# rainerzufalldererste/simd_dct

Hardware: AMD Instinct MI355X
Metric: Mpixels/s 8x8 fwd+inv int16 DCT, 8192x8192 plane (higher is better)
Workload: dtype f32

## Files before the change

simd_dct_amd/csrc/huffman_rows.h:

```cpp
#pragma once
#include <hip/hip_runtime.h>
#include "wg_sync.h"
#include <stdint.h>

namespace mdct
{

struct HuffArgs
{
  const int16_t *levels;
  const uint8_t *runs, *counts;
  uint8_t *out;
  uint32_t *seg_bytes;
  size_t seg_stride;
  uint32_t bpr, by0;
  uint32_t dc[12];
  uint32_t ac[256];
};

constexpr uint32_t kHuffRing = 2048;

__device__ __forceinline__ uint32_t ff_bytes(uint32_t w)
{
  const uint32_t t = ~w;
  return ~(((t & 0x7F7F7F7Fu) + 0x7F7F7F7Fu) | t | 0x7F7F7F7Fu);
}

struct HuffTok
{
  uint32_t bits, len;
};

__device__ __forceinline__ HuffTok huff_dc_token(int diff, const uint32_t *dc)
{
  diff = diff > 2047 ? 2047 : (diff < -2047 ? -2047 : diff);
  const int s = diff ? 32 - __builtin_clz((uint32_t)(diff < 0 ? -diff : diff)) : 0;
  const uint32_t e = dc[s];
  return {((e & 0xFFFFu) << s) | ((uint32_t)(diff < 0 ? diff - 1 : diff) & ((1u << s) - 1u)), (e >> 16) + (uint32_t)s};
}

__device__ __forceinline__ HuffTok huff_ac_token(int r, int l, const uint32_t *ac)
{
  l = l > 1023 ? 1023 : (l < -1023 ? -1023 : l);
  const int amp = l + (l >> 31);
  int lead;
  asm("v_ffbh_i32 %0, %1" : "=v"(lead) : "v"(amp));
  const int s = 32 - lead;
  const uint32_t e = ac[(r << 4) | s];
  return {((e & 0xFFFFu) << s) | ((uint32_t)amp & ((1u << s) - 1u)), (e >> 16) + (uint32_t)s};
}

template <int WAVES, int STAGE, bool TAIL, bool LATE_DC>
struct HuffRowCoder
{
  const uint32_t *ac, *dc;
  uint32_t *ring;
  uint32_t (*tot)[WAVES];
  int (*dcx)[2][WAVES];
  uint32_t *out_w;
  uint32_t zrl, eob;
  uint32_t bpr;
  uint32_t base_bits = 0;
  uint32_t par = 0;
  int carry_dc = 0;

  __device__ __forceinline__ void chunk(uint32_t c0, uint32_t *rec, int n, bool live, int prev_dc, const int16_t *lv_g, const uint8_t *rn_g)
  {
    constexpr uint32_t kChunk = 64 * WAVES;
    const uint32_t tid = threadIdx.x, lane = tid & 63, wave = tid >> 6;
    const int nl = n < STAGE ? n : STAGE;
    const uint32_t e0 = rec[0];
// ... 144 lines not shown
          put(eob & 0xFFFFu, eob >> 16);
        if (nacc && widx - win < kHuffRing)
          atomicOr(&ring[widx & (kHuffRing - 1)], acc << (32 - nacc));
      }
      wg_sync();
      const uint32_t stop = min(w_end, win + kHuffRing);
      for (uint32_t w = win + tid; w < stop; w += kChunk)
      {
        out_w[w] = __builtin_bswap32(ring[w & (kHuffRing - 1)]);
        ring[w & (kHuffRing - 1)] = 0;
      }
    }
    base_bits = end_bits;
    par ^= 1;
  }

  __device__ __forceinline__ uint32_t finish()
  {
    const uint32_t rem = base_bits & 31;
    if (rem)
    {
      const uint32_t pad = (8 - (rem & 7)) & 7;
      uint32_t w = ring[(base_bits >> 5) & (kHuffRing - 1)];
      if (pad)
        w |= ((1u << pad) - 1u) << (32 - rem - pad);
      out_w[base_bits >> 5] = __builtin_bswap32(w);
    }
    return (base_bits + 7) / 8;
  }
};

constexpr int kRec16Row = 66;

__device__ __forceinline__ HuffTok huff_ac_token12(uint32_t e, const uint32_t *ac)
{
  int l;
  asm("v_bfe_i32 %0, %1, 0, 12" : "=v"(l) : "v"(e));
  const int amp = l + (l >> 31);
  int lead;
  asm("v_ffbh_i32 %0, %1" : "=v"(lead) : "v"(amp));
  const int s = l ? 32 - lead : 0;
  const uint32_t c = ac[((e >> 12) << 4) | (uint32_t)s];
  return {((c & 0xFFFFu) << s) | ((uint32_t)amp & ((1u << s) - 1u)), (c >> 16) + (uint32_t)s};
}

template <int WAVES, uint32_t RING>
struct HuffRowCoder16
{
  const uint32_t *ac, *dc;
  uint32_t *ring;
  uint32_t (*tot)[WAVES];
  int (*dcx)[2][WAVES];
  uint32_t *out_w;
  uint32_t eob;
  uint32_t bpr;
  uint32_t base_bits = 0;
  uint32_t par = 0;
  int carry_dc = 0;
  uint32_t ff = 0;

  __device__ __forceinline__ void chunk(uint32_t c0, const uint16_t *rec, int n, bool live, int my_dc, bool need_eob)
  {
    constexpr uint32_t kChunk = 64 * WAVES;
    const uint32_t tid = threadIdx.x, lane = tid & 63, wave = tid >> 6;
    const uint32_t *rec2 = reinterpret_cast<const uint32_t *>(rec);
    if (!live)
    {
      my_dc = 0;
      n = 0;
    }
    const int up = __shfl_up(my_dc, 1, 64);
    HuffTok dct = huff_dc_token(my_dc - up, dc);
    if (lane == 0)
      dcx[par][0][wave] = my_dc;
    if (lane == 63)
      dcx[par][1][wave] = my_dc;
    uint32_t bits = 0;
    if (live)
    {
      bits = lane ? dct.len : 0u;
      for (int i = 0; i < n; i += 2)
      {
        const uint32_t w = rec2[i >> 1];
        bits += huff_ac_token12(w & 0xFFFFu, ac).len;
        if (i + 1 < n)
          bits += huff_ac_token12(w >> 16, ac).len;
      }
      if (need_eob)
        bits += eob >> 16;
    }
    uint32_t incl = bits;
#pragma unroll
    for (int d = 1; d < 64; d <<= 1)
    {
      const uint32_t v = __shfl_up(incl, d, 64);
      if (lane >= (uint32_t)d)
        incl += v;
    }
    if (lane == 63)
      tot[par][wave] = incl;
    wg_sync();
    uint32_t wave_start = 0, chunk_bits = 0, lane0_len = 0;
#pragma unroll
    for (uint32_t w = 0; w < (uint32_t)WAVES; w++)
    {
      const int pred = w == 0 ? (c0 == 0 ? 0 : carry_dc) : dcx[par][1][w - 1];
      const HuffTok t0 = huff_dc_token(dcx[par][0][w] - pred, dc);
      const uint32_t l0 = c0 + 64 * w < bpr ? t0.len : 0u;
      const uint32_t t = tot[par][w] + l0;
      if (w == wave)
      {
        lane0_len = l0;
        if (lane == 0)
          dct = t0;
      }
      wave_start += w < wave ? t : 0;
      chunk_bits += t;
    }
    carry_dc = dcx[par][1][WAVES - 1];
    const uint32_t end_bits = base_bits + chunk_bits;
    const uint32_t w_first = base_bits >> 5, w_end = end_bits >> 5;
    for (uint32_t win = w_first; win <= w_end; win += RING)
    {
      if (win != w_first)
      {
        wg_sync();
      }
      if (live)
      {
        const uint32_t cur = base_bits + wave_start + (incl - bits) + (lane ? lane0_len : 0u);
        uint32_t widx = cur >> 5;
        uint32_t acc = 0;
        uint32_t nacc = cur & 31;
        auto put = [&](uint32_t tok, uint32_t len) {
          const uint32_t total = nacc + len;
          if (total < 32)
          {
            acc = (acc << len) | tok;
            nacc = total;
          }
          else
          {
            const uint32_t over = total - 32;
            if (widx - win < RING)
              atomicOr(&ring[widx & (RING - 1)], (acc << ((32 - nacc) & 31)) | (tok >> over));
            widx++;
            acc = tok & ((1u << over) - 1u);
            nacc = over;
          }
        };
        put(dct.bits, dct.len);
        for (int i = 0; i < n; i += 2)
        {
          const uint32_t w = rec2[i >> 1];
          const HuffTok ta = huff_ac_token12(w & 0xFFFFu, ac);
          put(ta.bits, ta.len);
          if (i + 1 < n)
          {
            const HuffTok tb = huff_ac_token12(w >> 16, ac);
            put(tb.bits, tb.len);
          }
        }
        if (need_eob)
          put(eob & 0xFFFFu, eob >> 16);
        if (nacc && widx - win < RING)
          atomicOr(&ring[widx & (RING - 1)], acc << (32 - nacc));
      }
      wg_sync();
      const uint32_t stop = min(w_end, win + RING);
      for (uint32_t w = win + tid; w < stop; w += kChunk)
      {
        const uint32_t v = ring[w & (RING - 1)];
        ff += (uint32_t)__builtin_popcount(ff_bytes(v));
        out_w[w] = __builtin_bswap32(v);
        ring[w & (RING - 1)] = 0;
      }
    }
    base_bits = end_bits;
    par ^= 1;
  }

  __device__ __forceinline__ uint32_t finish(uint32_t *ff_last)
  {
    const uint32_t rem = base_bits & 31;
    *ff_last = 0;
    if (rem)
    {
      const uint32_t pad = (8 - (rem & 7)) & 7;
      uint32_t w = ring[(base_bits >> 5) & (RING - 1)];
      if (pad)
        w |= ((1u << pad) - 1u) << (32 - rem - pad);
      out_w[base_bits >> 5] = __builtin_bswap32(w);
      const uint32_t nbytes = (rem + 7) / 8;
      *ff_last = (uint32_t)__builtin_popcount(ff_bytes(w) & (0xFFFFFFFFu << (8 * (4 - nbytes))));
    }
    return (base_bits + 7) / 8;
  }
};

template <int WAVES, uint32_t RING>
struct HuffSeqCoder16
{
  uint32_t *ring;
  uint32_t (*tot)[WAVES];
  uint32_t *out_w;
  uint32_t base_bits = 0;
  uint32_t par = 0;
  uint32_t ff = 0;

  __device__ __forceinline__ void chunk(const uint16_t *rec, int n, bool live, int my_dc, int pred_dc, bool need_eob, const uint32_t *ac, const uint32_t *dc)
  {
    constexpr uint32_t kChunk = 64 * WAVES;
    const uint32_t tid = threadIdx.x, lane = tid & 63, wave = tid >> 6;
    const uint32_t *rec2 = reinterpret_cast<const uint32_t *>(rec);
    if (!live)
    {
      my_dc = pred_dc = 0;
      n = 0;
    }
    const HuffTok dct = huff_dc_token(my_dc - pred_dc, dc);
    const uint32_t eob = ac[0x00];
    uint32_t bits = 0;
    if (live)
    {
      bits = dct.len;
      for (int i = 0; i < n; i += 2)
      {
        const uint32_t w = rec2[i >> 1];
        bits += huff_ac_token12(w & 0xFFFFu, ac).len;
        if (i + 1 < n)
          bits += huff_ac_token12(w >> 16, ac).len;
      }
      if (need_eob)
        bits += eob >> 16;
    }
    uint32_t incl = bits;
#pragma unroll
    for (int d = 1; d < 64; d <<= 1)
    {
      const uint32_t v = __shfl_up(incl, d, 64);
      if (lane >= (uint32_t)d)
        incl += v;
    }
    if (lane == 63)
      tot[par][wave] = incl;
    wg_sync();
    uint32_t wave_start = 0, chunk_bits = 0;
#pragma unroll
    for (uint32_t w = 0; w < (uint32_t)WAVES; w++)
    {
      const uint32_t t = tot[par][w];
      wave_start += w < wave ? t : 0;
      chunk_bits += t;
    }
    const uint32_t end_bits = base_bits + chunk_bits;
    const uint32_t w_first = base_bits >> 5, w_end = end_bits >> 5;
    for (uint32_t win = w_first; win <= w_end; win += RING)
    {
      if (win != w_first)
        wg_sync();
      if (live)
      {
        const uint32_t cur = base_bits + wave_start + (incl - bits);
        uint32_t widx = cur >> 5;
        uint32_t acc = 0;
        uint32_t nacc = cur & 31;
        auto put = [&](uint32_t tok, uint32_t len) {
          const uint32_t total = nacc + len;
          if (total < 32)
          {
            acc = (acc << len) | tok;
            nacc = total;
          }
          else
          {
            const uint32_t over = total - 32;
            if (widx - win < RING)
              atomicOr(&ring[widx & (RING - 1)], (acc << ((32 - nacc) & 31)) | (tok >> over));
            widx++;
            acc = tok & ((1u << over) - 1u);
            nacc = over;
          }
        };
        put(dct.bits, dct.len);
        for (int i = 0; i < n; i += 2)
        {
          const uint32_t w = rec2[i >> 1];
          const HuffTok ta = huff_ac_token12(w & 0xFFFFu, ac);
          put(ta.bits, ta.len);
          if (i + 1 < n)
          {
            const HuffTok tb = huff_ac_token12(w >> 16, ac);
            put(tb.bits, tb.len);
          }
        }
        if (need_eob)
          put(eob & 0xFFFFu, eob >> 16);
        if (nacc && widx - win < RING)
          atomicOr(&ring[widx & (RING - 1)], acc << (32 - nacc));
      }
      wg_sync();
      const uint32_t stop = min(w_end, win + RING);
      for (uint32_t w = win + tid; w < stop; w += kChunk)
      {
        const uint32_t v = ring[w & (RING - 1)];
        ff += (uint32_t)__builtin_popcount(ff_bytes(v));
        out_w[w] = __builtin_bswap32(v);
        ring[w & (RING - 1)] = 0;
      }
    }
    base_bits = end_bits;
    par ^= 1;
  }

  __device__ __forceinline__ uint32_t finish(uint32_t *ff_last)
  {
    const uint32_t rem = base_bits & 31;
    *ff_last = 0;
    if (rem)
    {
      const uint32_t pad = (8 - (rem & 7)) & 7;
      uint32_t w = ring[(base_bits >> 5) & (RING - 1)];
      if (pad)
        w |= ((1u << pad) - 1u) << (32 - rem - pad);
      out_w[base_bits >> 5] = __builtin_bswap32(w);
      const uint32_t nbytes = (rem + 7) / 8;
      *ff_last = (uint32_t)__builtin_popcount(ff_bytes(w) & (0xFFFFFFFFu << (8 * (4 - nbytes))));
    }
    return (base_bits + 7) / 8;
  }
};

// ... 2 lines not shown
```

simd_dct_amd/csrc/mdct_kernels.hip:

```cpp
#include <hip/hip_runtime.h>
#include <stddef.h>
#include <stdint.h>
#include <stdlib.h>

#include <type_traits>

#include "wg_sync.h"
#include "huffman_rows.h"
#include "pack_rows.h"
#include "mdct_kernels.h"
#include "scan_records.h"
#include "aan_passes.h"

#pragma clang fp contract(off)

namespace mdct
{


enum { K_AVX = 0, K_SSE = 1, K_TRUE = 2 };

__device__ __forceinline__ void aan_fwd8(const DctConsts &C, float &p0, float &p1, float &p2, float &p3, float &p4, float &p5, float &p6, float &p7)
{
  const float t0 = p0 + p7, t7 = p0 - p7, t1 = p1 + p6, t6 = p1 - p6;
// ... 809 lines not shown
__device__ __forceinline__ void quant_dequant8(const AanPk &K, f32x2 (&p)[8], const f32x2 (&qf)[8], const f32x2 (&dq)[8])
{
#define MDCT_Q8(OP, A, B, MOD) OP " %0, %0, " A "0" B MOD OP " %1, %1, " A "1" B MOD OP " %2, %2, " A "2" B MOD OP " %3, %3, " A "3" B MOD OP " %4, %4, " A "4" B MOD OP " %5, %5, " A "5" B MOD OP " %6, %6, " A "6" B MOD OP " %7, %7, " A "7" B MOD
  asm("v_pk_fma_f32 %0, %0, %8, %24 op_sel:[0,0,0] op_sel_hi:[1,1,0]\n\t"
      "v_pk_fma_f32 %1, %1, %9, %24 op_sel:[0,0,0] op_sel_hi:[1,1,0]\n\t"
      "v_pk_fma_f32 %2, %2, %10, %24 op_sel:[0,0,0] op_sel_hi:[1,1,0]\n\t"
      "v_pk_fma_f32 %3, %3, %11, %24 op_sel:[0,0,0] op_sel_hi:[1,1,0]\n\t"
      "v_pk_fma_f32 %4, %4, %12, %24 op_sel:[0,0,0] op_sel_hi:[1,1,0]\n\t"
      "v_pk_fma_f32 %5, %5, %13, %24 op_sel:[0,0,0] op_sel_hi:[1,1,0]\n\t"
      "v_pk_fma_f32 %6, %6, %14, %24 op_sel:[0,0,0] op_sel_hi:[1,1,0]\n\t"
      "v_pk_fma_f32 %7, %7, %15, %24 op_sel:[0,0,0] op_sel_hi:[1,1,0]\n\t"
      "v_pk_add_f32 %0, %0, %24 op_sel:[0,0] op_sel_hi:[1,0] neg_lo:[0,1] neg_hi:[0,1]\n\t"
      "v_pk_add_f32 %1, %1, %24 op_sel:[0,0] op_sel_hi:[1,0] neg_lo:[0,1] neg_hi:[0,1]\n\t"
      "v_pk_add_f32 %2, %2, %24 op_sel:[0,0] op_sel_hi:[1,0] neg_lo:[0,1] neg_hi:[0,1]\n\t"
      "v_pk_add_f32 %3, %3, %24 op_sel:[0,0] op_sel_hi:[1,0] neg_lo:[0,1] neg_hi:[0,1]\n\t"
      "v_pk_add_f32 %4, %4, %24 op_sel:[0,0] op_sel_hi:[1,0] neg_lo:[0,1] neg_hi:[0,1]\n\t"
      "v_pk_add_f32 %5, %5, %24 op_sel:[0,0] op_sel_hi:[1,0] neg_lo:[0,1] neg_hi:[0,1]\n\t"
      "v_pk_add_f32 %6, %6, %24 op_sel:[0,0] op_sel_hi:[1,0] neg_lo:[0,1] neg_hi:[0,1]\n\t"
      "v_pk_add_f32 %7, %7, %24 op_sel:[0,0] op_sel_hi:[1,0] neg_lo:[0,1] neg_hi:[0,1]\n\t"
      "v_pk_mul_f32 %0, %0, %16 op_sel:[0,0] op_sel_hi:[1,1]\n\t"
      "v_pk_mul_f32 %1, %1, %17 op_sel:[0,0] op_sel_hi:[1,1]\n\t"
      "v_pk_mul_f32 %2, %2, %18 op_sel:[0,0] op_sel_hi:[1,1]\n\t"
      "v_pk_mul_f32 %3, %3, %19 op_sel:[0,0] op_sel_hi:[1,1]\n\t"
      "v_pk_mul_f32 %4, %4, %20 op_sel:[0,0] op_sel_hi:[1,1]\n\t"
      "v_pk_mul_f32 %5, %5, %21 op_sel:[0,0] op_sel_hi:[1,1]\n\t"
      "v_pk_mul_f32 %6, %6, %22 op_sel:[0,0] op_sel_hi:[1,1]\n\t"
      "v_pk_mul_f32 %7, %7, %23 op_sel:[0,0] op_sel_hi:[1,1]"
      : "+v"(p[0]), "+v"(p[1]), "+v"(p[2]), "+v"(p[3]), "+v"(p[4]), "+v"(p[5]), "+v"(p[6]), "+v"(p[7])
      : "s"(qf[0]), "s"(qf[1]), "s"(qf[2]), "s"(qf[3]), "s"(qf[4]), "s"(qf[5]), "s"(qf[6]), "s"(qf[7]), "s"(dq[0]), "s"(dq[1]), "s"(dq[2]), "s"(dq[3]), "s"(dq[4]), "s"(dq[5]),
        "s"(dq[6]), "s"(dq[7]), "v"(K.magic));
#undef MDCT_Q8
}

template <bool HAS_LUT, class Rows, bool PRIO = false, bool SAT = true>
__device__ __forceinline__ void i16_roundtrip_rows(const DctConsts &C, const Rows rows, kbytes_t tbp);

__device__ __forceinline__ kbytes_t const_bytes(const void *p)
{
  const uint64_t v = (uint64_t)p;
  const uint32_t lo = __builtin_amdgcn_readfirstlane((uint32_t)v), hi = __builtin_amdgcn_readfirstlane((uint32_t)(v >> 32));
  return (kbytes_t)(((uint64_t)hi << 32) | lo);
}

template <bool SAT>
__device__ __forceinline__ void quant_dequant_pairs(const AanPk &K, f32x2 (&p)[8], karg_pairs_t tq, karg_pairs_t td)
{
  if constexpr (!SAT)
  {
    const f32x2 qf[8] = {tq[0], tq[1], tq[2], tq[3], tq[4], tq[5], tq[6], tq[7]}, dq[8] = {td[0], td[1], td[2], td[3], td[4], td[5], td[6], td[7]};
    quant_dequant8(K, p, qf, dq);
  }
  else
  {
    const f32x2 magic_v = K.magic;
#pragma unroll
    for (int v = 0; v < 8; v++)
    {
      const f32x2 qf = tq[v], dq = td[v];
      f32x2 m;
      MDCT_PKF(m, p[v], qf, magic_v, "op_sel:[0,0,0] op_sel_hi:[1,1,0]");
      if constexpr (SAT)
      {
        m.x = __builtin_amdgcn_fmed3f(m.x, kQLo, kQHi);
        m.y = __builtin_amdgcn_fmed3f(m.y, kQLo, kQHi);
      }
      MDCT_PKA(m, m, K.magic, MDCT_K_LL " " MDCT_NEG_B);
      MDCT_PKM(p[v], m, dq, MDCT_K_LH);
    }
  }
}

template <bool HAS_LUT, class Rows, bool PRIO, bool SAT>
__device__ __forceinline__ void i16_roundtrip_rows(const DctConsts &C, const Rows rows, kbytes_t tbp)
{
  const AanPk &K = reinterpret_cast<const AanPk &>(C);
  uint4 in[8];
#pragma unroll
  for (int r = 0; r < 8; r++)
    in[r] = rows.ld(r);
  MDCT_PHASE_PRIO(1);
  f32x2 P[4][8];
#pragma unroll
  for (int r = 0; r < 8; r++)
  {
    const f32x2 a01 = {(float)(int16_t)(in[r].x & 0xFFFF), (float)(int16_t)(in[r].x >> 16)};
    const f32x2 a23 = {(float)(int16_t)(in[r].y & 0xFFFF), (float)(int16_t)(in[r].y >> 16)};
    const f32x2 a45 = {(float)(int16_t)(in[r].z & 0xFFFF), (float)(int16_t)(in[r].z >> 16)};
    const f32x2 a67 = {(float)(int16_t)(in[r].w & 0xFFFF), (float)(int16_t)(in[r].w >> 16)};
    aan_fwd_h(K, a01, a23, a45, a67, P[0][r], P[1][r], P[2][r], P[3][r]);
  }
  MDCT_PHASE_PRIO(2);
#pragma unroll
  for (int j = 0; j < 4; j++)
  {
    aan_fwd_v(K, P[j]);
    if constexpr (HAS_LUT)
    {
      karg_pairs_t tq = (karg_pairs_t)(tbp + offsetof(OwnTables, qf)) + j * 8, td = (karg_pairs_t)(tbp + offsetof(OwnTables, dq)) + j * 8;
      asm volatile("" : "+s"(tq), "+s"(td));
      quant_dequant_pairs<SAT>(K, P[j], tq, td);
    }
    aan_inv_v(K, P[j]);
  }
  MDCT_PHASE_PRIO(3);
  constexpr float scale = HAS_LUT ? 1.0f : 64.0f;
#pragma unroll
  for (int r = 0; r < 8; r++)
  {
    f32x2 o07, o16, o25, o43;
    aan_inv_h(K, P[0][r], P[1][r], P[2][r], P[3][r], o07, o16, o25, o43);
    auto fin = [&](f32x2 v) {
      f32x2 t;
      v.x = __builtin_amdgcn_fmed3f(v.x, -32768.0f * scale, 32767.0f * scale);
      v.y = __builtin_amdgcn_fmed3f(v.y, -32768.0f * scale, 32767.0f * scale);
      if constexpr (HAS_LUT)
        MDCT_PKA(t, v, K.magic, MDCT_K_LL);
      else
        MDCT_PKA(t, v, K.magic, MDCT_K_HH);
      return t;
    };
    const f32x2 b07 = fin(o07), b16 = fin(o16), b25 = fin(o25), b43 = fin(o43);
    rows.st(r, pack_lo16(__float_as_uint(b07.x), __float_as_uint(b16.x)), pack_lo16(__float_as_uint(b25.x), __float_as_uint(b43.y)),
            pack_lo16(__float_as_uint(b43.x), __float_as_uint(b25.y)), pack_lo16(__float_as_uint(b16.y), __float_as_uint(b07.y)));
  }
}

typedef const __attribute__((address_space(4))) OwnTables *ktables_t;
__device__ __forceinline__ kbytes_t i16_tables(const I16Args &a) { return a.tb_dev ? const_bytes(a.tb_dev) : karg_bytes(offsetof(I16Args, tb)); }

constexpr int i16_waves(int mode) { return mode == MODE_ROUNDTRIP ? 3 : (mode == MODE_FWD ? 2 : 4); }
template <int MODE, bool HAS_LUT, bool SAT = true>
__global__ __launch_bounds__(kWG) __attribute__((amdgpu_waves_per_eu(i16_waves(MODE), i16_waves(MODE)))) void k_i16(I16Args a)
{
  const uint32_t t = wg_index() * kWG + threadIdx.x;
  if (t >= a.nblocks)
    return;
  const uint32_t row = t / a.bpr;
  const uint32_t bx = t - row * a.bpr;
  const size_t by = a.by0 + row;
  const int16_t *src = a.from + by * 8 * a.pitch_in + (size_t)bx * 8;
  int16_t *dst = a.to + by * 8 * a.pitch_out + (size_t)bx * 8;
  const kbytes_t tbp = i16_tables(a);
  if constexpr (MODE == MODE_ROUNDTRIP)
    i16_roundtrip_rows<HAS_LUT, RowsLinear, false, SAT>(a.consts, RowsLinear{src, dst, a.pitch_in, a.pitch_out}, tbp);
  else
    i16_block<MODE, HAS_LUT>(a.consts, RowsLinear{src, dst, a.pitch_in, a.pitch_out}, *(ktables_t)tbp);
}

constexpr uint32_t kTileSmallLaunch = 6144;
template <int MODE, bool HAS_LUT, bool SAT = true, int WAVES = 2>
__global__ __launch_bounds__(64) __attribute__((amdgpu_waves_per_eu(WAVES, WAVES))) void k_i16_tile(I16Args a)
{
  const size_t by = a.by0 + blockIdx.y;
  const RowsTiled rows{a.from + by * 8 * a.pitch_in + (size_t)blockIdx.x * 512, a.to + by * 8 * a.pitch_out + (size_t)blockIdx.x * 512, a.pitch_in, a.pitch_out, threadIdx.x * 16, threadIdx.x * 16};
  const kbytes_t tbp = i16_tables(a);
  if constexpr (MODE == MODE_ROUNDTRIP)
    i16_roundtrip_rows<HAS_LUT, RowsTiled, true, SAT>(a.consts, rows, tbp);
  else
    i16_block<MODE, HAS_LUT>(a.consts, rows, *(ktables_t)tbp);
}

// ... 26 lines not shown
  const u32x16_s h = *(const __attribute__((address_space(4))) u32x16_s *)args;
  const u32x4_s ptrs = *(const __attribute__((address_space(4))) u32x4_s *)(args + offsetof(BatchArgs, descs));
  const uint32_t n = h[0], uniform = h[1], pp_m = h[2], pp_s = h[3], table_bytes = h[4];
  const uint64_t descs_dev = ((uint64_t)ptrs[1] << 32) | ptrs[0], tables_dev = ((uint64_t)ptrs[3] << 32) | ptrs[2];
  const kbytes_t blob = args + offsetof(BatchArgs, blob);
  const kbytes_t descs = descs_dev ? (kbytes_t)descs_dev : blob + table_bytes;
  const kbytes_t tables = tables_dev ? (kbytes_t)tables_dev : blob;
  const uint32_t first8[kBatchChain] = {h[8], h[9], h[10], h[11], h[12], h[13], h[14], h[15]};
  static_assert(kBatchChain == 8 && offsetof(BatchHead, first8) == 32, "first8 = dwords 8..15 of the header");
  uint32_t p = batch_plane_of(w, n, uniform, pp_m, pp_s, first8, [descs](uint32_t k) {
    return *(const __attribute__((address_space(4))) uint32_t *)(descs + (size_t)k * sizeof(BatchDesc) + offsetof(BatchDesc, first));
  });
  p = __builtin_amdgcn_readfirstlane(p);
  kbytes_t dp = descs + (size_t)p * sizeof(BatchDesc);
  asm volatile("" : "+s"(dp));
  BatchTile t;
  t.d = *(const __attribute__((address_space(4))) u32x16_s *)dp;
  const uint32_t lt = w - t.d[12];
  if constexpr (PAIRS)
  {
    const BatchPos at = batch_pos(lt, t.d[8], t.d[9], t.d[10], t.d[11], t.d[14], t.d[15]);
    t.row = at.row, t.b0 = at.b0, t.s = at.s, t.straddle = at.straddle, t.tile = at.b0 >> 6;
  }
  else
  {
    t.row = magic_apply(lt, t.d[10], t.d[11]);
    t.tile = lt - t.row * t.d[9];
    t.b0 = t.tile * 64, t.s = 64, t.straddle = 0;
  }
  t.tables = tables + t.d[13];
  return t;
}

constexpr int batch_waves(int mode) { return mode == MODE_ROUNDTRIP ? 3 : 2; }
template <int MODE, int LUTMODE, bool SAT = true, bool SMALL = false>
__global__ __launch_bounds__(64) __attribute__((amdgpu_waves_per_eu(SMALL ? 4 : batch_waves(MODE), SMALL ? 4 : batch_waves(MODE)))) void k_i16_batch(BatchArgs a)
{
  const BatchTile t = batch_tile<true>(blockIdx.x);
  if (!t.straddle && threadIdx.x >= t.s)
    return;
  const size_t pin = t.pitch_in(), pout = t.pitch_out();
  const uint32_t hop = (t.straddle && threadIdx.x >= t.s) ? 0xFFFFFFFFu : 0u;
  const RowsTiled rows{(const int16_t *)t.from() + (size_t)t.row * 8 * pin + (size_t)t.b0 * 8, (int16_t *)t.to() + (size_t)t.row * 8 * pout + (size_t)t.b0 * 8, pin, pout,
                       threadIdx.x * 16 + (hop & (((uint32_t)pin - t.bpr()) * 16)), threadIdx.x * 16 + (hop & (((uint32_t)pout - t.bpr()) * 16))};
  if constexpr (MODE == MODE_ROUNDTRIP)
  {
    if (LUTMODE == BATCH_ALL_LUT || (LUTMODE == BATCH_MIXED && t.has_lut()))
      i16_roundtrip_rows<true, RowsTiled, true, SAT>(a.consts, rows, t.tables);
    else
      i16_roundtrip_rows<false, RowsTiled, true>(a.consts, rows, nullptr);
  }
  else
    i16_block<MODE, true>(a.consts, rows, *(ktables_t)t.tables);
}

__device__ __forceinline__ uint32_t pack4_sat_u8(float x0, float x1, float x2, float x3)
{
  uint32_t w = __builtin_amdgcn_cvt_pk_u8_f32(x0, 0, 0u);
  w = __builtin_amdgcn_cvt_pk_u8_f32(x1, 1, w);
  w = __builtin_amdgcn_cvt_pk_u8_f32(x2, 2, w);
  return __builtin_amdgcn_cvt_pk_u8_f32(x3, 3, w);
}
enum { U8_RT = 0, U8_FWD = 1, U8_INV = 2 };
template <int MODE, bool SAT, bool PRIO>
__device__ __forceinline__ void u8_rows(const DctConsts &C, const f32x2 shifts, const void *src, void *dst, size_t pitch_in, size_t pitch_out, uint32_t in_off, uint32_t out_off, kbytes_t tbp)
{
  const AanPk &K = reinterpret_cast<const AanPk &>(C);
  f32x2 P[4][8];
  if constexpr (MODE != U8_INV)
  {
    uint2 rows[8];
    load_block_rows_g(static_cast<const uint8_t *>(src), pitch_in, in_off, rows);
    MDCT_PHASE_PRIO(1);
#pragma unroll
    for (int r = 0; r < 8; r++)
    {
      const f32x2 a01 = {ubyte_to_float<0>(rows[r].x), ubyte_to_float<1>(rows[r].x)}, a23 = {ubyte_to_float<2>(rows[r].x), ubyte_to_float<3>(rows[r].x)};
      const f32x2 a45 = {ubyte_to_float<0>(rows[r].y), ubyte_to_float<1>(rows[r].y)}, a67 = {ubyte_to_float<2>(rows[r].y), ubyte_to_float<3>(rows[r].y)};
      aan_fwd_h(K, a01, a23, a45, a67, P[0][r], P[1][r], P[2][r], P[3][r]);
    }
  }
// ... 258 lines not shown
  __shared__ uint32_t ac[256], dc[12];
  __shared__ __attribute__((aligned(16))) uint16_t rec_all[WAVES][64 * kRec16Row];
  static_assert(!PACK || sizeof(rec_all) >= kPackStageWords * 4, "the packing tail stages a window in the record rows");
  __shared__ uint32_t ring[kFusedRing];
  __shared__ uint32_t tot[2][WAVES];
  __shared__ int dcx[2][2][WAVES];
  __shared__ uint32_t ff_total;
  constexpr uint32_t kChunk = 64 * WAVES;
  const uint32_t tid = threadIdx.x, lane = tid & 63, wave = tid >> 6;
  const uint32_t row = a.by0 + blockIdx.x;
  uint32_t tag = 0;
  if constexpr (PACK)
  {
    if (chain_failed(a.work))
    {
      if (tid == 0)
      {
        a.row_off[blockIdx.x] = ~0ull;
        if (blockIdx.x + 1 == a.n_rows)
          a.row_off[a.n_rows] = ~0ull;
      }
      return;
    }
    tag = __builtin_amdgcn_readfirstlane(chain_epoch_tag(a.work));
  }
  for (uint32_t i = tid; i < 256; i += kChunk)
    ac[i] = a.ac[i];
  if (tid < 12)
    dc[tid] = a.dc[tid];
  if (tid == 0)
    ff_total = 0;
  for (uint32_t w = tid; w < kFusedRing; w += kChunk)
    ring[w] = 0;
  HuffRowCoder16<WAVES, kFusedRing> coder;
  coder.ac = ac;
  coder.dc = dc;
  coder.ring = ring;
  coder.tot = tot;
  coder.dcx = dcx;
  coder.out_w = reinterpret_cast<uint32_t *>(a.out + (size_t)row * a.seg_stride);
  coder.eob = a.ac[0x00];
  coder.bpr = a.bpr;
  const DctConsts &C = a.consts;
  const AanPk &K = reinterpret_cast<const AanPk &>(C);
  uint16_t *rec = rec_all[wave] + lane * kRec16Row;
  const uint32_t last_blk = a.bpr - 1;

  typedef typename std::conditional<I16_IN, uint4, uint2>::type row_t;
  row_t rows[8];
  auto fetch = [&](uint32_t bx) {
    const uint32_t blk = min(bx, last_blk);
    if constexpr (I16_IN)
    {
      const int16_t *src = reinterpret_cast<const int16_t *>(a.px) + (size_t)row * 8 * a.pitch_px + (size_t)blk * 8;
#pragma unroll
      for (int r = 0; r < 8; r++)
        rows[r] = ld_stream16(src + (size_t)r * a.pitch_px);
    }
    else
    {
      const uint8_t *src = a.px + (size_t)row * 8 * a.pitch_px + (size_t)blk * 8;
#pragma unroll
      for (int r = 0; r < 8; r++)
        rows[r] = load8(src + (size_t)r * a.pitch_px);
    }
  };
  fetch(wave * 64 + lane);
// ... 601 lines not shown
```

simd_dct_amd/csrc/mdct_kernels.h:

```cpp
#ifndef MDCT_KERNELS_H
#define MDCT_KERNELS_H

#include <hip/hip_runtime.h>
#include <stddef.h>
#include <stdint.h>

#include "mdct.h"
#include "batch_plan.h"
#include "launch_tally.h"

namespace mdct
{

enum { MODE_FWD = 0, MODE_INV = 1, MODE_ROUNDTRIP = 2 };

struct DctConsts
{
  float c707 = 0.707106781186547524f;
  float c382 = 0.382683432365089772f;
  float c541 = 0.541196100146196985f;
  float c1306 = 1.306562964876376528f;
  float c1414 = 1.414213562373095049f;
  float c1847 = 1.847759065022573512f;
  float c1082 = 1.082392200292393968f;
// ... 23 lines not shown
struct PkConstsArg
{
  float af[2], cd[2], be[2], nm[2];
  float da[2], fd[2], fc[2], ca[2];
  float bias[2];
  float div[2];
};

struct U8Args
{
  const uint8_t *from;
  uint8_t *to;
  QuantTable qt;
  PkConstsArg pk;
  DctConsts consts;
  size_t pitch;
  size_t sizeX;
  size_t out_strip;
  size_t eye_offset;
  size_t plane_stride;
  uint32_t bpr;
  uint32_t by0;
  uint32_t by_last;
  uint32_t nblocks;
  uint32_t spill_ok;
  uint32_t out_tight;
};

struct I16Args
{
  const int16_t *from;
  int16_t *to;
  const OwnTables *tb_dev;
  OwnTables tb;
  DctConsts consts;
  size_t pitch_in, pitch_out;
  uint32_t bpr, by0, nblocks;
};

struct U8I16Args
{
  const uint8_t *px;
  int16_t *coef;
  OwnTables tb;
  DctConsts consts;
  size_t pitch_px, pitch_coef;
  uint32_t bpr, by0, nblocks;
  float dc_shift;
};

struct U8RecArgs
{
  const uint8_t *px;
  int16_t *levels;
  uint8_t *runs;
  uint8_t *counts;
  OwnTables tb;
  DctConsts consts;
  size_t pitch_px;
  uint32_t bpr, by0, nblocks;
  float dc_shift;
};

struct PxHuffArgs
{
  const uint8_t *px;
  uint8_t *out;
  uint32_t *seg_bytes;
  uint32_t *ff_counts;
  size_t seg_stride;
  size_t pitch_px;
// ... 67 lines not shown
```

Baseline: 1.561 million.

## Cache Huffman tokens in registers and streamline bit packing and scans

Rewrites the Huffman row coders so the first group of AC tokens computed in the counting pass is kept in registers and reused in the emit pass, avoiding a second table lookup. The shuffle-based wave prefix sum becomes a DPP scan, per-wave DC tokens are computed one per lane and gathered with readlane, and the bit packer uses a 64-bit shift with alignbit plus a window-free path when the chunk fits in the ring. The DC and AC size computations also use a branchless ffbh trick. The cost is higher register pressure from the token arrays, which could lower occupancy; the fused kernel uses a smaller token cache for int16 input.

```diff
diff --git a/simd_dct_amd/csrc/huffman_rows.h b/simd_dct_amd/csrc/huffman_rows.h
--- a/simd_dct_amd/csrc/huffman_rows.h
+++ b/simd_dct_amd/csrc/huffman_rows.h
@@ -34,9 +34,12 @@
 __device__ __forceinline__ HuffTok huff_dc_token(int diff, const uint32_t *dc)
 {
   diff = diff > 2047 ? 2047 : (diff < -2047 ? -2047 : diff);
-  const int s = diff ? 32 - __builtin_clz((uint32_t)(diff < 0 ? -diff : diff)) : 0;
+  const int amp = diff + (diff >> 31);
+  int lead;
+  asm("v_ffbh_i32 %0, %1" : "=v"(lead) : "v"(amp << 1 | 1));
+  const int s = 31 - lead;
   const uint32_t e = dc[s];
-  return {((e & 0xFFFFu) << s) | ((uint32_t)(diff < 0 ? diff - 1 : diff) & ((1u << s) - 1u)), (e >> 16) + (uint32_t)s};
+  return {((e & 0xFFFFu) << s) | ((uint32_t)amp & ((1u << s) - 1u)), (e >> 16) + (uint32_t)s};
 }
 
 __device__ __forceinline__ HuffTok huff_ac_token(int r, int l, const uint32_t *ac)
@@ -247,19 +250,150 @@
 
 constexpr int kRec16Row = 66;
 
+__device__ __forceinline__ HuffTok huff_ac_token_rl(uint32_t run, int l, const uint32_t *ac)
+{
+  const int amp = l + (l >> 31);
+  int lead;
+  asm("v_ffbh_i32 %0, %1" : "=v"(lead) : "v"(amp << 1 | 1));
+  const int s = 31 - lead;
+  const uint32_t c = ac[(run << 4) | (uint32_t)s];
+  return {((c & 0xFFFFu) << s) | ((uint32_t)amp & ((1u << s) - 1u)), (c >> 16) + (uint32_t)s};
+}
+
 __device__ __forceinline__ HuffTok huff_ac_token12(uint32_t e, const uint32_t *ac)
 {
   int l;
   asm("v_bfe_i32 %0, %1, 0, 12" : "=v"(l) : "v"(e));
-  const int amp = l + (l >> 31);
-  int lead;
-  asm("v_ffbh_i32 %0, %1" : "=v"(lead) : "v"(amp));
-  const int s = l ? 32 - lead : 0;
-  const uint32_t c = ac[((e >> 12) << 4) | (uint32_t)s];
-  return {((c & 0xFFFFu) << s) | ((uint32_t)amp & ((1u << s) - 1u)), (c >> 16) + (uint32_t)s};
-}
-
-template <int WAVES, uint32_t RING>
+  return huff_ac_token_rl(e >> 12, l, ac);
+}
+
+template <int HALF>
+__device__ __forceinline__ HuffTok huff_ac_token12h(uint32_t w, const uint32_t *ac)
+{
+  int l;
+  if (HALF)
+    asm("v_bfe_i32 %0, %1, 16, 12" : "=v"(l) : "v"(w));
+  else
+    asm("v_bfe_i32 %0, %1, 0, 12" : "=v"(l) : "v"(w));
+  return huff_ac_token_rl(HALF ? w >> 28 : (w >> 12) & 15u, l, ac);
+}
+
+constexpr int kTokRegs = 16;
+
+template <int TOKS>
+struct EntryToks
+{
+  static_assert(TOKS % 4 == 0 && TOKS <= 64, "whole groups, inside the row");
+  uint32_t bits[TOKS], len[TOKS];
+};
+
+template <int TOKS>
+__device__ __forceinline__ uint32_t count_entries16(const uint32_t *rec2, int n, const uint32_t *ac, EntryToks<TOKS> &tk)
+{
+  uint32_t bits = 0;
+#pragma unroll
+  for (int g = 0; g < TOKS / 4; g++)
+  {
+    if (__builtin_amdgcn_ballot_w64(4 * g < n))
+    {
+#pragma unroll
+      for (int j = 2 * g; j < 2 * g + 2; j++)
+      {
+        const uint32_t w = rec2[j];
+        const HuffTok ta = huff_ac_token12h<0>(w, ac), tb = huff_ac_token12h<1>(w, ac);
+        const bool va = 2 * j < n, vb = 2 * j + 1 < n;
+        tk.bits[2 * j] = va ? ta.bits : 0u;
+        tk.len[2 * j] = va ? ta.len : 0u;
+        tk.bits[2 * j + 1] = vb ? tb.bits : 0u;
+        tk.len[2 * j + 1] = vb ? tb.len : 0u;
+        bits += tk.len[2 * j] + tk.len[2 * j + 1];
+      }
+    }
+    else
+    {
+#pragma unroll
+      for (int i = 4 * g; i < 4 * g + 4; i++)
+        tk.bits[i] = tk.len[i] = 0;
+    }
+  }
+  for (int i = TOKS; i < n; i += 2)
+  {
+    const uint32_t w = rec2[i >> 1];
+    bits += huff_ac_token12h<0>(w, ac).len;
+    if (i + 1 < n)
+      bits += huff_ac_token12h<1>(w, ac).len;
+  }
+  return bits;
+}
+
+__device__ __forceinline__ uint32_t wave_scan_incl(uint32_t v)
+{
+  v += (uint32_t)__builtin_amdgcn_update_dpp(0, (int)v, 0x111, 0xF, 0xF, false);
+  v += (uint32_t)__builtin_amdgcn_update_dpp(0, (int)v, 0x112, 0xF, 0xF, false);
+  v += (uint32_t)__builtin_amdgcn_update_dpp(0, (int)v, 0x114, 0xF, 0xF, false);
+  v += (uint32_t)__builtin_amdgcn_update_dpp(0, (int)v, 0x118, 0xF, 0xF, false);
+  v += (uint32_t)__builtin_amdgcn_update_dpp(0, (int)v, 0x142, 0xA, 0xF, false);
+  v += (uint32_t)__builtin_amdgcn_update_dpp(0, (int)v, 0x143, 0xC, 0xF, false);
+  return v;
+}
+
+template <uint32_t RING, bool WINDOWS>
+struct RingPut
+{
+  uint32_t *ring;
+  uint32_t win4, at4, nacc, lo, hi;
+
+  __device__ __forceinline__ RingPut(uint32_t *ring_, uint32_t win, uint32_t cur) : ring(ring_), win4(win * 4), at4((cur >> 5) * 4), nacc(cur & 31), lo(0), hi(0) {}
+
+  __device__ __forceinline__ uint32_t *slot() const { return reinterpret_cast<uint32_t *>(reinterpret_cast<char *>(ring) + (at4 & (RING * 4 - 4))); }
+
+  __device__ __forceinline__ void put(uint32_t tok, uint32_t len)
+  {
+    const unsigned long long t = ((unsigned long long)hi << 32 | lo) << len;
+    hi = (uint32_t)(t >> 32);
+    lo = (uint32_t)t | tok;
+    nacc += len;
+    if (nacc >= 32)
+    {
+      nacc -= 32;
+      if (!WINDOWS || at4 - win4 < RING * 4)
+        atomicOr(slot(), __builtin_amdgcn_alignbit(hi, lo, nacc));
+      at4 += 4;
+    }
+  }
+
+  __device__ __forceinline__ void flush()
+  {
+    if (nacc && (!WINDOWS || at4 - win4 < RING * 4))
+      atomicOr(slot(), lo << (32 - nacc));
+  }
+};
+
+template <uint32_t RING, bool WINDOWS, int TOKS>
+__device__ __forceinline__ void emit_entries16(RingPut<RING, WINDOWS> &out, const uint32_t *rec2, int n, const uint32_t *ac, const EntryToks<TOKS> &tk)
+{
+#pragma unroll
+  for (int g = 0; g < TOKS / 4; g++)
+    if (__builtin_amdgcn_ballot_w64(4 * g < n))
+    {
+#pragma unroll
+      for (int i = 4 * g; i < 4 * g + 4; i++)
+        out.put(tk.bits[i], tk.len[i]);
+    }
+  for (int i = TOKS; i < n; i += 2)
+  {
+    const uint32_t w = rec2[i >> 1];
+    const HuffTok ta = huff_ac_token12h<0>(w, ac);
+    out.put(ta.bits, ta.len);
+    if (i + 1 < n)
+    {
+      const HuffTok tb = huff_ac_token12h<1>(w, ac);
+      out.put(tb.bits, tb.len);
+    }
+  }
+}
+
+template <int WAVES, uint32_t RING, int TOKS = kTokRegs>
 struct HuffRowCoder16
 {
   const uint32_t *ac, *dc;
@@ -277,7 +411,7 @@
   __device__ __forceinline__ void chunk(uint32_t c0, const uint16_t *rec, int n, bool live, int my_dc, bool need_eob)
   {
     constexpr uint32_t kChunk = 64 * WAVES;
-    const uint32_t tid = threadIdx.x, lane = tid & 63, wave = tid >> 6;
+    const uint32_t tid = threadIdx.x, lane = tid & 63, wave = __builtin_amdgcn_readfirstlane(tid >> 6);
     const uint32_t *rec2 = reinterpret_cast<const uint32_t *>(rec);
     if (!live)
     {
@@ -290,47 +424,39 @@
       dcx[par][0][wave] = my_dc;
     if (lane == 63)
       dcx[par][1][wave] = my_dc;
-    uint32_t bits = 0;
+    EntryToks<TOKS> tk;
+    uint32_t bits = count_entries16(rec2, n, ac, tk);
     if (live)
     {
-      bits = lane ? dct.len : 0u;
-      for (int i = 0; i < n; i += 2)
-      {
-        const uint32_t w = rec2[i >> 1];
-        bits += huff_ac_token12(w & 0xFFFFu, ac).len;
-        if (i + 1 < n)
-          bits += huff_ac_token12(w >> 16, ac).len;
-      }
+      bits += lane ? dct.len : 0u;
       if (need_eob)
         bits += eob >> 16;
     }
-    uint32_t incl = bits;
-#pragma unroll
-    for (int d = 1; d < 64; d <<= 1)
-    {
-      const uint32_t v = __shfl_up(incl, d, 64);
-      if (lane >= (uint32_t)d)
-        incl += v;
-    }
+    const uint32_t incl = wave_scan_incl(bits);
     if (lane == 63)
       tot[par][wave] = incl;
     wg_sync();
-    uint32_t wave_start = 0, chunk_bits = 0, lane0_len = 0;
+    static_assert(WAVES <= 64, "one lane per wave");
+    uint32_t wl = lane;
+    asm volatile("" : "+v"(wl));
+    wl = min(wl, (uint32_t)WAVES - 1u);
+    const int prev_last = dcx[par][1][wl ? wl - 1u : 0u];
+    const HuffTok t0 = huff_dc_token(dcx[par][0][wl] - (wl ? prev_last : (c0 == 0 ? 0 : carry_dc)), dc);
+    const uint32_t l0 = c0 + 64 * wl < bpr ? t0.len : 0u;
+    const uint32_t tw = tot[par][wl] + l0;
+    uint32_t wave_start = 0, chunk_bits = 0;
 #pragma unroll
     for (uint32_t w = 0; w < (uint32_t)WAVES; w++)
     {
-      const int pred = w == 0 ? (c0 == 0 ? 0 : carry_dc) : dcx[par][1][w - 1];
-      const HuffTok t0 = huff_dc_token(dcx[par][0][w] - pred, dc);
-      const uint32_t l0 = c0 + 64 * w < bpr ? t0.len : 0u;
-      const uint32_t t = tot[par][w] + l0;
-      if (w == wave)
-      {
-        lane0_len = l0;
-        if (lane == 0)
-          dct = t0;
-      }
+      const uint32_t t = __builtin_amdgcn_readlane(tw, w);
       wave_start += w < wave ? t : 0;
       chunk_bits += t;
+    }
+    const uint32_t lane0_len = __builtin_amdgcn_readlane(l0, wave);
+    {
+      const uint32_t b0 = __builtin_amdgcn_readlane(t0.bits, wave), n0 = __builtin_amdgcn_readlane(t0.len, wave);
+      if (lane == 0)
+        dct = {b0, n0};
     }
     carry_dc = dcx[par][1][WAVES - 1];
     const uint32_t end_bits = base_bits + chunk_bits;
@@ -344,42 +470,17 @@
       if (live)
       {
         const uint32_t cur = base_bits + wave_start + (incl - bits) + (lane ? lane0_len : 0u);
-        uint32_t widx = cur >> 5;
-        uint32_t acc = 0;
-        uint32_t nacc = cur & 31;
-        auto put = [&](uint32_t tok, uint32_t len) {
-          const uint32_t total = nacc + len;
-          if (total < 32)
-          {
-            acc = (acc << len) | tok;
-            nacc = total;
-          }
-          else
-          {
-            const uint32_t over = total - 32;
-            if (widx - win < RING)
-              atomicOr(&ring[widx & (RING - 1)], (acc << ((32 - nacc) & 31)) | (tok >> over));
-            widx++;
-            acc = tok & ((1u << over) - 1u);
-            nacc = over;
-          }
+        auto emit = [&](auto out) {
+          out.put(dct.bits, dct.len);
+          emit_entries16(out, rec2, n, ac, tk);
+          if (need_eob)
+            out.put(eob & 0xFFFFu, eob >> 16);
+          out.flush();
         };
-        put(dct.bits, dct.len);
-        for (int i = 0; i < n; i += 2)
-        {
-          const uint32_t w = rec2[i >> 1];
-          const HuffTok ta = huff_ac_token12(w & 0xFFFFu, ac);
-          put(ta.bits, ta.len);
-          if (i + 1 < n)
-          {
-            const HuffTok tb = huff_ac_token12(w >> 16, ac);
-            put(tb.bits, tb.len);
-          }
-        }
-        if (need_eob)
-          put(eob & 0xFFFFu, eob >> 16);
-        if (nacc && widx - win < RING)
-          atomicOr(&ring[widx & (RING - 1)], acc << (32 - nacc));
+        if (w_end - w_first < RING)
+          emit(RingPut<RING, false>(ring, win, cur));
+        else
+          emit(RingPut<RING, true>(ring, win, cur));
       }
       wg_sync();
       const uint32_t stop = min(w_end, win + RING);
@@ -413,7 +514,7 @@
   }
 };
 
-template <int WAVES, uint32_t RING>
+template <int WAVES, uint32_t RING, int TOKS = kTokRegs>
 struct HuffSeqCoder16
 {
   uint32_t *ring;
@@ -435,28 +536,15 @@
     }
     const HuffTok dct = huff_dc_token(my_dc - pred_dc, dc);
     const uint32_t eob = ac[0x00];
-    uint32_t bits = 0;
+    EntryToks<TOKS> tk;
+    uint32_t bits = count_entries16(rec2, n, ac, tk);
     if (live)
     {
-      bits = dct.len;
-      for (int i = 0; i < n; i += 2)
-      {
-        const uint32_t w = rec2[i >> 1];
-        bits += huff_ac_token12(w & 0xFFFFu, ac).len;
-        if (i + 1 < n)
-          bits += huff_ac_token12(w >> 16, ac).len;
-      }
+      bits += dct.len;
       if (need_eob)
         bits += eob >> 16;
     }
-    uint32_t incl = bits;
-#pragma unroll
-    for (int d = 1; d < 64; d <<= 1)
-    {
-      const uint32_t v = __shfl_up(incl, d, 64);
-      if (lane >= (uint32_t)d)
-        incl += v;
-    }
+    const uint32_t incl = wave_scan_incl(bits);
     if (lane == 63)
       tot[par][wave] = incl;
     wg_sync();
@@ -477,42 +565,17 @@
       if (live)
       {
         const uint32_t cur = base_bits + wave_start + (incl - bits);
-        uint32_t widx = cur >> 5;
-        uint32_t acc = 0;
-        uint32_t nacc = cur & 31;
-        auto put = [&](uint32_t tok, uint32_t len) {
-          const uint32_t total = nacc + len;
-          if (total < 32)
-          {
-            acc = (acc << len) | tok;
-            nacc = total;
-          }
-          else
-          {
-            const uint32_t over = total - 32;
-            if (widx - win < RING)
-              atomicOr(&ring[widx & (RING - 1)], (acc << ((32 - nacc) & 31)) | (tok >> over));
-            widx++;
-            acc = tok & ((1u << over) - 1u);
-            nacc = over;
-          }
+        auto emit = [&](auto out) {
+          out.put(dct.bits, dct.len);
+          emit_entries16(out, rec2, n, ac, tk);
+          if (need_eob)
+            out.put(eob & 0xFFFFu, eob >> 16);
+          out.flush();
         };
-        put(dct.bits, dct.len);
-        for (int i = 0; i < n; i += 2)
-        {
-          const uint32_t w = rec2[i >> 1];
-          const HuffTok ta = huff_ac_token12(w & 0xFFFFu, ac);
-          put(ta.bits, ta.len);
-          if (i + 1 < n)
-          {
-            const HuffTok tb = huff_ac_token12(w >> 16, ac);
-            put(tb.bits, tb.len);
-          }
-        }
-        if (need_eob)
-          put(eob & 0xFFFFu, eob >> 16);
-        if (nacc && widx - win < RING)
-          atomicOr(&ring[widx & (RING - 1)], acc << (32 - nacc));
+        if (w_end - w_first < RING)
+          emit(RingPut<RING, false>(ring, win, cur));
+        else
+          emit(RingPut<RING, true>(ring, win, cur));
       }
       wg_sync();
       const uint32_t stop = min(w_end, win + RING);
diff --git a/simd_dct_amd/csrc/mdct_kernels.hip b/simd_dct_amd/csrc/mdct_kernels.hip
--- a/simd_dct_amd/csrc/mdct_kernels.hip
+++ b/simd_dct_amd/csrc/mdct_kernels.hip
@@ -1391,7 +1391,7 @@
     ff_total = 0;
   for (uint32_t w = tid; w < kFusedRing; w += kChunk)
     ring[w] = 0;
-  HuffRowCoder16<WAVES, kFusedRing> coder;
+  HuffRowCoder16<WAVES, kFusedRing, I16_IN ? 8 : kTokRegs> coder;
   coder.ac = ac;
   coder.dc = dc;
   coder.ring = ring;
```

Result: no change. 1.560 million (-0.0%).

## Prefetch quant tables into scalar registers ahead of the roundtrip compute

Applied to the files above, without the earlier changes.

Loads the quantise/dequantise table pairs for the first two column groups before the forward pass starts. The tables for later groups are loaded double-buffered after each quantise step, so scalar-load latency overlaps with the vector DCT math. It also reorders I16Args so pointers, counts and constants sit in the first 128 bytes with the tables aligned at 128. It drops the readfirstlane on the device table pointer and lowers the waves-per-EU target for the all-LUT batch roundtrip kernel to 2. The extra prefetched tables raise scalar register pressure, which the lower occupancy target is meant to make room for.

```diff
diff --git a/simd_dct_amd/csrc/mdct_kernels.h b/simd_dct_amd/csrc/mdct_kernels.h
--- a/simd_dct_amd/csrc/mdct_kernels.h
+++ b/simd_dct_amd/csrc/mdct_kernels.h
@@ -79,11 +79,13 @@
   const int16_t *from;
   int16_t *to;
   const OwnTables *tb_dev;
-  OwnTables tb;
-  DctConsts consts;
   size_t pitch_in, pitch_out;
   uint32_t bpr, by0, nblocks;
+  DctConsts consts;
+  alignas(64) OwnTables tb;
 };
+static_assert(offsetof(I16Args, nblocks) + sizeof(uint32_t) <= 64 && offsetof(I16Args, consts) + sizeof(DctConsts) <= 128 && offsetof(I16Args, tb) == 128,
+              "pointers, pitches and counts in the first 64 bytes, the constants in the next, the embedded tables last");
 
 struct U8I16Args
 {
diff --git a/simd_dct_amd/csrc/mdct_kernels.hip b/simd_dct_amd/csrc/mdct_kernels.hip
--- a/simd_dct_amd/csrc/mdct_kernels.hip
+++ b/simd_dct_amd/csrc/mdct_kernels.hip
@@ -865,7 +865,7 @@
 #undef MDCT_Q8
 }
 
-template <bool HAS_LUT, class Rows, bool PRIO = false, bool SAT = true>
+template <bool HAS_LUT, class Rows, bool PRIO = false, bool SAT = true, bool AHEAD = true>
 __device__ __forceinline__ void i16_roundtrip_rows(const DctConsts &C, const Rows rows, kbytes_t tbp);
 
 __device__ __forceinline__ kbytes_t const_bytes(const void *p)
@@ -876,34 +876,50 @@
 }
 
 template <bool SAT>
+__device__ __forceinline__ void quant_dequant_regs(const AanPk &K, f32x2 (&p)[8], const f32x2 (&qf)[8], const f32x2 (&dq)[8])
+{
+  if constexpr (!SAT)
+    quant_dequant8(K, p, qf, dq);
+  else
+  {
+    const f32x2 magic_v = K.magic;
+#pragma unroll
+    for (int v = 0; v < 8; v++)
+    {
+      f32x2 m;
+      MDCT_PKF(m, p[v], qf[v], magic_v, "op_sel:[0,0,0] op_sel_hi:[1,1,0]");
+      m.x = __builtin_amdgcn_fmed3f(m.x, kQLo, kQHi);
+      m.y = __builtin_amdgcn_fmed3f(m.y, kQLo, kQHi);
+      MDCT_PKA(m, m, K.magic, MDCT_K_LL " " MDCT_NEG_B);
+      MDCT_PKM(p[v], m, dq[v], MDCT_K_LH);
+    }
+  }
+}
+template <bool SAT>
 __device__ __forceinline__ void quant_dequant_pairs(const AanPk &K, f32x2 (&p)[8], karg_pairs_t tq, karg_pairs_t td)
 {
-  if constexpr (!SAT)
-  {
-    const f32x2 qf[8] = {tq[0], tq[1], tq[2], tq[3], tq[4], tq[5], tq[6], tq[7]}, dq[8] = {td[0], td[1], td[2], td[3], td[4], td[5], td[6], td[7]};
-    quant_dequant8(K, p, qf, dq);
-  }
-  else
-  {
-    const f32x2 magic_v = K.magic;
-#pragma unroll
-    for (int v = 0; v < 8; v++)
-    {
-      const f32x2 qf = tq[v], dq = td[v];
-      f32x2 m;
-      MDCT_PKF(m, p[v], qf, magic_v, "op_sel:[0,0,0] op_sel_hi:[1,1,0]");
-      if constexpr (SAT)
-      {
-        m.x = __builtin_amdgcn_fmed3f(m.x, kQLo, kQHi);
-        m.y = __builtin_amdgcn_fmed3f(m.y, kQLo, kQHi);
-      }
-      MDCT_PKA(m, m, K.magic, MDCT_K_LL " " MDCT_NEG_B);
-      MDCT_PKM(p[v], m, dq, MDCT_K_LH);
-    }
-  }
-}
-
-template <bool HAS_LUT, class Rows, bool PRIO, bool SAT>
+  const f32x2 qf[8] = {tq[0], tq[1], tq[2], tq[3], tq[4], tq[5], tq[6], tq[7]}, dq[8] = {td[0], td[1], td[2], td[3], td[4], td[5], td[6], td[7]};
+  quant_dequant_regs<SAT>(K, p, qf, dq);
+}
+
+__device__ __forceinline__ void load_pair_tables(kbytes_t tbp, int j, f32x2 (&qf)[8], f32x2 (&dq)[8])
+{
+  karg_pairs_t tq = (karg_pairs_t)(tbp + offsetof(OwnTables, qf)) + j * 8, td = (karg_pairs_t)(tbp + offsetof(OwnTables, dq)) + j * 8;
+  asm volatile("" : "+s"(tq), "+s"(td));
+#pragma unroll
+  for (int v = 0; v < 8; v++)
+    qf[v] = tq[v], dq[v] = td[v];
+}
+__device__ __forceinline__ void load_pair_tables_after(kbytes_t tbp, int j, f32x2 (&qf)[8], f32x2 (&dq)[8], const f32x2 (&after)[8])
+{
+  karg_pairs_t tq = (karg_pairs_t)(tbp + offsetof(OwnTables, qf)) + j * 8, td = (karg_pairs_t)(tbp + offsetof(OwnTables, dq)) + j * 8;
+  asm volatile("" : "+s"(tq), "+s"(td) : "v"(after[0]), "v"(after[1]), "v"(after[2]), "v"(after[3]), "v"(after[4]), "v"(after[5]), "v"(after[6]), "v"(after[7]));
+#pragma unroll
+  for (int v = 0; v < 8; v++)
+    qf[v] = tq[v], dq[v] = td[v];
+}
+
+template <bool HAS_LUT, class Rows, bool PRIO, bool SAT, bool AHEAD>
 __device__ __forceinline__ void i16_roundtrip_rows(const DctConsts &C, const Rows rows, kbytes_t tbp)
 {
   const AanPk &K = reinterpret_cast<const AanPk &>(C);
@@ -911,6 +927,14 @@
 #pragma unroll
   for (int r = 0; r < 8; r++)
     in[r] = rows.ld(r);
+  [[maybe_unused]] f32x2 qfa[8], dqa[8], qfb[8], dqb[8];
+  if constexpr (HAS_LUT && AHEAD)
+  {
+    if constexpr (PRIO)
+      __builtin_amdgcn_sched_barrier(0);
+    load_pair_tables(tbp, 0, qfa, dqa);
+    load_pair_tables(tbp, 1, qfb, dqb);
+  }
   MDCT_PHASE_PRIO(1);
   f32x2 P[4][8];
 #pragma unroll
@@ -927,11 +951,24 @@
   for (int j = 0; j < 4; j++)
   {
     aan_fwd_v(K, P[j]);
-    if constexpr (HAS_LUT)
+    if constexpr (HAS_LUT && !AHEAD)
     {
       karg_pairs_t tq = (karg_pairs_t)(tbp + offsetof(OwnTables, qf)) + j * 8, td = (karg_pairs_t)(tbp + offsetof(OwnTables, dq)) + j * 8;
       asm volatile("" : "+s"(tq), "+s"(td));
       quant_dequant_pairs<SAT>(K, P[j], tq, td);
+    }
+    else if constexpr (HAS_LUT)
+    {
+      if (j & 1)
+        quant_dequant_regs<SAT>(K, P[j], qfb, dqb);
+      else
+        quant_dequant_regs<SAT>(K, P[j], qfa, dqa);
+      if (j == 0)
+        load_pair_tables_after(tbp, 2, qfa, dqa, P[0]);
+      if (j == 1)
+        load_pair_tables_after(tbp, 3, qfb, dqb, P[1]);
+      if (j < 2)
+        __builtin_amdgcn_sched_barrier(0);
     }
     aan_inv_v(K, P[j]);
   }
@@ -959,7 +996,7 @@
 }
 
 typedef const __attribute__((address_space(4))) OwnTables *ktables_t;
-__device__ __forceinline__ kbytes_t i16_tables(const I16Args &a) { return a.tb_dev ? const_bytes(a.tb_dev) : karg_bytes(offsetof(I16Args, tb)); }
+__device__ __forceinline__ kbytes_t i16_tables(const I16Args &a) { return a.tb_dev ? (kbytes_t)(uint64_t)a.tb_dev : karg_bytes(offsetof(I16Args, tb)); }
 
 constexpr int i16_waves(int mode) { return mode == MODE_ROUNDTRIP ? 3 : (mode == MODE_FWD ? 2 : 4); }
 template <int MODE, bool HAS_LUT, bool SAT = true>
@@ -1052,9 +1089,12 @@
   return t;
 }
 
-constexpr int batch_waves(int mode) { return mode == MODE_ROUNDTRIP ? 3 : 2; }
+#ifndef MDCT_I16_BATCH_LUT_WAVES
+#define MDCT_I16_BATCH_LUT_WAVES 2
+#endif
+constexpr int batch_waves(int mode, int lutmode) { return mode == MODE_ROUNDTRIP ? (lutmode == BATCH_ALL_LUT ? MDCT_I16_BATCH_LUT_WAVES : 3) : 2; }
 template <int MODE, int LUTMODE, bool SAT = true, bool SMALL = false>
-__global__ __launch_bounds__(64) __attribute__((amdgpu_waves_per_eu(SMALL ? 4 : batch_waves(MODE), SMALL ? 4 : batch_waves(MODE)))) void k_i16_batch(BatchArgs a)
+__global__ __launch_bounds__(64) __attribute__((amdgpu_waves_per_eu(SMALL ? 4 : batch_waves(MODE, LUTMODE), SMALL ? 4 : batch_waves(MODE, LUTMODE)))) void k_i16_batch(BatchArgs a)
 {
   const BatchTile t = batch_tile<true>(blockIdx.x);
   if (!t.straddle && threadIdx.x >= t.s)
@@ -1066,7 +1106,7 @@
   if constexpr (MODE == MODE_ROUNDTRIP)
   {
     if (LUTMODE == BATCH_ALL_LUT || (LUTMODE == BATCH_MIXED && t.has_lut()))
-      i16_roundtrip_rows<true, RowsTiled, true, SAT>(a.consts, rows, t.tables);
+      i16_roundtrip_rows<true, RowsTiled, true, SAT, LUTMODE == BATCH_ALL_LUT>(a.consts, rows, t.tables);
     else
       i16_roundtrip_rows<false, RowsTiled, true>(a.consts, rows, nullptr);
   }
```

Result: slower. 1.564 million before, 1.124 million after (-28.2%).
